# andrewjong/SwapNet

Measured on AMD Instinct MI355X. Metric: images/sec full G+D step, warp-stage 256x256 bs=32/GPU, higher is better.
Workload: dtype f32; 1 GPU; warp-stage G+D optimize_parameters step, 256x256, bs 32/GPU, fp32 storage and accumulation, GEMM products on the 16-bit MFMA pipe from operand splits: forward / input-gradient GEMMs as 2 fp16 planes of amax-scaled operands (22 of 24 mantissa bits, 3 of 4 terms, the dropped one below 2^-22), weight-gradient GEMMs in the same two-plane form, train mode (dropout 0.5), WarpModule 137.6M + PatchGAN 2.8; step_form=eager launches, global_batch=32, parallelism=dp1

## Files before the change

### swapnet_amd/csrc/wino.hip

```cpp
#include "hip_util.h"

namespace swn {
namespace {

__device__ __forceinline__ float4 f4add(float4 a, float4 b) { return make_float4(a.x + b.x, a.y + b.y, a.z + b.z, a.w + b.w); }
__device__ __forceinline__ float4 f4sub(float4 a, float4 b) { return make_float4(a.x - b.x, a.y - b.y, a.z - b.z, a.w - b.w); }

__device__ __forceinline__ int wsrc(int e, int ext, int pad_mode) {
  if (pad_mode == PAD_REFLECT) {
    if (e < 0) e = -e;
    else if (e >= ext) e = 2 * ext - 2 - e;
    return e;
  }
  return (e < 0 || e >= ext) ? -1 : e;
}

__global__ __launch_bounds__(256) void wino_input_kernel(const float* x, int xcs, int N, int H, int W, int C, int pad,
                                                         int pad_mode, int Th, int Tw, float* V) {
  const int C4 = C >> 2;
  const size_t T = (size_t)N * Th * Tw;
  const size_t total = T * C4;
  for (size_t i = (size_t)blockIdx.x * 256 + threadIdx.x; i < total; i += (size_t)gridDim.x * 256) {
    const size_t tile = i / C4;
    const int c = (int)(i - tile * C4) * 4;
// ... 378 lines not shown
#pragma unroll
    for (int b = 0; b < A; ++b) {
      float4 m[A];
#pragma unroll
      for (int a = 0; a < A; ++a) m[a] = *reinterpret_cast<const float4*>(Mx + ((size_t)(a * A + b) * T + tile) * Cm + c);
#pragma unroll
      for (int r = 0; r < M; ++r) {
        float4 s = F4ZERO;
#pragma unroll
        for (int k = 0; k < A; ++k) f4mac(s, F::AT[r][k], m[k]);
        s1[r][b] = s;
      }
    }
    float4 bv = F4ZERO;
    if (bias) bv = make_float4(c < Cout ? bias[c] : 0.f, c + 1 < Cout ? bias[c + 1] : 0.f,
                               c + 2 < Cout ? bias[c + 2] : 0.f, c + 3 < Cout ? bias[c + 3] : 0.f);
#pragma unroll
    for (int a = 0; a < M; ++a)
#pragma unroll
      for (int b = 0; b < M; ++b) {
        const int oy = M * ty + a, ox = M * tx + b;
        if (oy >= yH || ox >= yW) continue;
        float4 v = F4ZERO;
#pragma unroll
        for (int k = 0; k < A; ++k) f4mac(v, F::AT[b][k], s1[a][k]);
        v = f4add(v, bv);
        v.x = act_apply(v.x, act); v.y = act_apply(v.y, act); v.z = act_apply(v.z, act); v.w = act_apply(v.w, act);
        float* dst = y + ((size_t)(n * yH + oy) * yW + ox) * ycs + c;
        if (accumulate) v = f4add(v, *reinterpret_cast<const float4*>(dst));
        if (c + 3 < Cout) {
          *reinterpret_cast<float4*>(dst) = v;
          amx = fmaxf(amx, fmaxf(fmaxf(fabsf(v.x), fabsf(v.y)), fmaxf(fabsf(v.z), fabsf(v.w))));
        } else {
          const float vv[4] = {v.x, v.y, v.z, v.w};
          for (int j = 0; j < 4 && c + j < Cout; ++j) { dst[j] = vv[j]; amx = fmaxf(amx, fabsf(vv[j])); }
        }
      }
  }
  amax_fold(amx, amax_out);
}

template <class F, int VW>
__global__ __launch_bounds__(256) void winog_dy_kernel(const float* dy, int dcs, int N, int H, int W, int C, int Th, int Tw,
                                                       float* dM, float* amax_out, const float* in_amax, float gain, int* kscale_out) {
  constexpr int A = F::A, M = F::M;
  typedef fvec<VW> vt;
  const int Cv = C / VW;
  const size_t T = (size_t)N * Th * Tw;
  const size_t total = T * Cv;
  float am = 0.f;
  const bool pair = in_amax != nullptr;
  const float psc = pair ? __uint_as_float((unsigned)(127 + pair_scale_exp(in_amax, gain, kscale_out)) << 23) : 1.f;
  for (size_t i = (size_t)blockIdx.x * 256 + threadIdx.x; i < total; i += (size_t)gridDim.x * 256) {
    const size_t tile = i / Cv;
    const int c = (int)(i - tile * Cv) * VW;
    const int tx = (int)(tile % Tw); size_t q = tile / Tw;
    const int ty = (int)(q % Th); const int n = (int)(q / Th);
    vt r[A][M];
#pragma unroll
    for (int b = 0; b < M; ++b) {
      vt g[M];
#pragma unroll
      for (int a = 0; a < M; ++a) {
        const int oy = M * ty + a, ox = M * tx + b;
        g[a] = (oy < H && ox < W) ? *reinterpret_cast<const vt*>(dy + ((size_t)(n * H + oy) * W + ox) * dcs + c) : vt(0.f);
      }
#pragma unroll
      for (int p = 0; p < A; ++p) {
        vt s = vt(0.f);
#pragma unroll
        for (int a = 0; a < M; ++a)
          if (F::AT[a][p] != 0.f) s += F::AT[a][p] * g[a];
        r[p][b] = s;
      }
    }
#pragma unroll
    for (int p = 0; p < A; ++p)
#pragma unroll
      for (int j = 0; j < A; ++j) {
        vt s = vt(0.f);
#pragma unroll
        for (int b = 0; b < M; ++b)
          if (F::AT[b][j] != 0.f) s += F::AT[b][j] * r[p][b];
        *reinterpret_cast<vt*>(dM + ((size_t)(p * A + j) * T + tile) * C + c) = pair ? pairv<VW>(s, psc) : s;
        am = fmaxf(am, fvamax<VW>(s));
      }
  }
  if (!pair) amax_fold(am, amax_out);
}

template <class F>
__global__ __launch_bounds__(256) void winog_filter_grad_kernel(WShape w, const float* dU, float* dpacked) {
  constexpr int A = F::A, R = F::R;
  const size_t total = (size_t)w.Cip * w.Npad;
  const size_t i = (size_t)blockIdx.x * 256 + threadIdx.x;
  if (i >= total) return;
  float t[R][A];
#pragma unroll
  for (int b = 0; b < A; ++b) {
    float u[A];
#pragma unroll
    for (int a = 0; a < A; ++a) u[a] = dU[(size_t)(a * A + b) * total + i];
#pragma unroll
    for (int r = 0; r < R; ++r) {
      float s = 0.f;
#pragma unroll
      for (int a = 0; a < A; ++a) f1mac(s, F::G[a][r], u[a]);
      t[r][b] = s;
    }
  }
#pragma unroll
  for (int a = 0; a < R; ++a)
#pragma unroll
    for (int j = 0; j < R; ++j) {
      float s = 0.f;
#pragma unroll
      for (int b = 0; b < A; ++b) f1mac(s, F::G[b][j], t[a][b]);
      dpacked[(size_t)(a * R + j) * total + i] = s;
    }
}


struct F23 {
  static constexpr int M = 2, R = 3, A = 4;
  static constexpr float BT[4][4] = {{1, 0, -1, 0}, {0, 1, 1, 0}, {0, -1, 1, 0}, {0, 1, 0, -1}};
};

template <class F>
__global__ __launch_bounds__(256) void winog_patch_kernel(float* V, int C, size_t T) {
  constexpr int A = F::A;
  const int C4 = C >> 2;
  const size_t total = T * C4;
  for (size_t i = (size_t)blockIdx.x * 256 + threadIdx.x; i < total; i += (size_t)gridDim.x * 256) {
    const size_t tile = i / C4;
    const int c = (int)(i - tile * C4) * 4;
    float4 t[A][A];
#pragma unroll
    for (int b = 0; b < A; ++b) {
      float4 v[A];
#pragma unroll
      for (int a = 0; a < A; ++a) v[a] = *reinterpret_cast<const float4*>(V + ((size_t)(a * A + b) * T + tile) * C + c);
#pragma unroll
      for (int r = 0; r < A; ++r) {
        float4 s = F4ZERO;
#pragma unroll
        for (int k = 0; k < A; ++k) f4mac(s, F::BT[k][r], v[k]);
        t[r][b] = s;
      }
    }
#pragma unroll
    for (int a = 0; a < A; ++a)
#pragma unroll
      for (int j = 0; j < A; ++j) {
        float4 s = F4ZERO;
#pragma unroll
        for (int k = 0; k < A; ++k) f4mac(s, F::BT[k][j], t[a][k]);
        *reinterpret_cast<float4*>(V + ((size_t)(a * A + j) * T + tile) * C + c) = s;
      }
  }
}

__device__ __forceinline__ int adj_sources(int y, int ext, int pad, int pad_mode, int emax, int (&e)[3]) {
  int n = 0;
  if (y <= emax) e[n++] = y;
  if (pad_mode == PAD_REFLECT) {
    if (y >= 1 && -y >= -pad) e[n++] = -y;
    const int r = 2 * ext - 2 - y;
    if (r >= ext && r <= emax) e[n++] = r;
  }
  return n;
}

__global__ __launch_bounds__(256) void wino_fold_kernel(const float* P, int C, int N, int H, int W, int m, int A, int pad,
                                                        int pad_mode, int Th, int Tw, float* dx, int dcs, int accumulate) {
  const int C4 = C >> 2;
  const size_t T = (size_t)N * Th * Tw;
  const size_t total = (size_t)N * H * W * C4;
  const int emax_y = m * (Th - 1) - pad + A - 1, emax_x = m * (Tw - 1) - pad + A - 1;
  for (size_t i = (size_t)blockIdx.x * 256 + threadIdx.x; i < total; i += (size_t)gridDim.x * 256) {
    const size_t px = i / C4;
    const int c = (int)(i - px * C4) * 4;
    const int n = (int)(px / ((size_t)H * W));
    const int rem = (int)(px - (size_t)n * H * W);
    const int y = rem / W, x = rem - y * W;
    int ey[3], ex[3];
    const int ny = adj_sources(y, H, pad, pad_mode, emax_y, ey), nx = adj_sources(x, W, pad, pad_mode, emax_x, ex);
    float4 acc = F4ZERO;
    for (int iy = 0; iy < ny; ++iy) {
      const int qy = ey[iy] + pad;
      const int ty1 = min(qy / m, Th - 1);
      for (int ty = ty1; ty >= 0 && qy - m * ty < A; --ty) {
        const int a = qy - m * ty;
        for (int ix = 0; ix < nx; ++ix) {
          const int qx = ex[ix] + pad;
          const int tx1 = min(qx / m, Tw - 1);
          for (int tx = tx1; tx >= 0 && qx - m * tx < A; --tx) {
            const int b = qx - m * tx;
            const size_t tile = ((size_t)n * Th + ty) * Tw + tx;
            const float4 v = *reinterpret_cast<const float4*>(P + ((size_t)(a * A + b) * T + tile) * C + c);
            acc = f4add(acc, v);
          }
        }
      }
    }
    float* d = dx + px * dcs + c;
    if (accumulate) acc = f4add(acc, *reinterpret_cast<const float4*>(d));
    *reinterpret_cast<float4*>(d) = acc;
  }
}


struct F42 {
  static constexpr int M = 4, R = 2, A = 5;
  static constexpr float BT[5][5] = {{0.5f, -1, -0.5f, 1, 0}, {0, -0.5f, 0.5f, 1, 0}, {0, 0.5f, -1.5f, 1, 0}, {0, -1, 0, 1, 0},
                                     {0, 0.5f, -1, -0.5f, 1}};
  static constexpr float G[5][2] = {{2, 0}, {1, 1}, {-1.f / 3, 1.f / 3}, {-8.f / 3, -4.f / 3}, {0, 1}};
  static constexpr float AT[4][5] = {{1, 1, 1, 1, 0}, {0, 1, -1, 0.5f, 0}, {0, 1, 1, 0.25f, 0}, {0, 1, -1, 0.125f, 1}};
};

template <int VW>
__global__ __launch_bounds__(256) void wino_s2_input_kernel(const float* x, int xcs, int N, int H, int W, int C, int Th, int Tw,
                                                            float* V, float* amax_out, const float* in_amax, float gain, int* kscale_out) {
  constexpr int A = 5;
  typedef fvec<VW> vt;
  const int C4 = C / VW;
  const size_t T = (size_t)N * Th * Tw;
  const size_t total = T * 4 * C4;
  const int CV = 4 * C;
  float am = 0.f;
  const bool pair = in_amax != nullptr;
  const float psc = pair ? __uint_as_float((unsigned)(127 + pair_scale_exp(in_amax, gain, kscale_out)) << 23) : 1.f;
  for (size_t i = (size_t)blockIdx.x * 256 + threadIdx.x; i < total; i += (size_t)gridDim.x * 256) {
    const int c = (int)(i % C4) * VW; size_t r = i / C4;
    const int q = (int)(r & 3); const size_t tile = r >> 2;
    const int s = q >> 1, t = q & 1;
    const int tx = (int)(tile % Tw); size_t u = tile / Tw;
    const int ty = (int)(u % Th); const int n = (int)(u / Th);
    int sy[A];
#pragma unroll
    for (int a = 0; a < A; ++a) { const int e = 2 * (4 * ty + a) - 1 + s; sy[a] = (e >= 0 && e < H) ? e : -1; }
    vt tt[A][A];
#pragma unroll
    for (int b = 0; b < A; ++b) {
      const int e = 2 * (4 * tx + b) - 1 + t;
      const int sx = (e >= 0 && e < W) ? e : -1;
      vt d[A];
#pragma unroll
      for (int a = 0; a < A; ++a)
        d[a] = (sy[a] >= 0 && sx >= 0) ? *reinterpret_cast<const vt*>(x + ((size_t)(n * H + sy[a]) * W + sx) * xcs + c) : vt(0.f);
#pragma unroll
      for (int rr = 0; rr < A; ++rr) {
        vt acc = vt(0.f);
#pragma unroll
        for (int k = 0; k < A; ++k)
          if (F42::BT[rr][k] != 0.f) acc += F42::BT[rr][k] * d[k];
        tt[rr][b] = acc;
      }
    }
#pragma unroll
    for (int a = 0; a < A; ++a)
#pragma unroll
      for (int j = 0; j < A; ++j) {
        vt acc = vt(0.f);
#pragma unroll
        for (int k = 0; k < A; ++k)
          if (F42::BT[j][k] != 0.f) acc += F42::BT[j][k] * tt[a][k];
        *reinterpret_cast<vt*>(V + ((size_t)(a * A + j) * T + tile) * CV + q * C + c) = pair ? pairv<VW>(acc, psc) : acc;
        am = fmaxf(am, fvamax<VW>(acc));
      }
  }
  if (!pair) amax_fold(am, amax_out);
}

__global__ __launch_bounds__(256) void wino_s2_fold_kernel(const float* P, int C, int N, int H, int W, int Th, int Tw, const float* bias,
                                                           float* dx, int dcs, int accumulate) {
  constexpr int A = 5, M = 4;
  const int C4 = C >> 2, CV = 4 * C;
  const size_t T = (size_t)N * Th * Tw;
  const size_t total = (size_t)N * H * W * C4;
  for (size_t i = (size_t)blockIdx.x * 256 + threadIdx.x; i < total; i += (size_t)gridDim.x * 256) {
    const size_t px = i / C4;
    const int c = (int)(i - px * C4) * 4;
    const int n = (int)(px / ((size_t)H * W));
    const int rem = (int)(px - (size_t)n * H * W);
    const int r = rem / W, cc = rem - r * W;
    const int s = (r + 1) & 1, t = (cc + 1) & 1;
    const int qy = (r + 1 - s) >> 1, qx = (cc + 1 - t) >> 1;
    float4 acc = F4ZERO;
    for (int ty = min(qy / M, Th - 1); ty >= 0 && qy - M * ty < A; --ty) {
      const int a = qy - M * ty;
      for (int tx = min(qx / M, Tw - 1); tx >= 0 && qx - M * tx < A; --tx) {
        const int b = qx - M * tx;
        const size_t tile = ((size_t)n * Th + ty) * Tw + tx;
        acc = f4add(acc, *reinterpret_cast<const float4*>(P + ((size_t)(a * A + b) * T + tile) * CV + (2 * s + t) * C + c));
      }
    }
    if (bias) { acc.x += bias[c]; acc.y += bias[c + 1]; acc.z += bias[c + 2]; acc.w += bias[c + 3]; }
    float* d = dx + px * dcs + c;
    if (accumulate) acc = f4add(acc, *reinterpret_cast<const float4*>(d));
    *reinterpret_cast<float4*>(d) = acc;
  }
}

__device__ __forceinline__ size_t s2_widx(const WShape& w, int kh, int kw, int cf, int cc) {
  if (w.kind == WK_CONV) return ((size_t)(kh * 4 + kw) * w.Cip + cf) * w.Npad + cc;
  const int a = (3 - kh) & 1, dy = (3 - kh - a) >> 1, b = (3 - kw) & 1, dx = (3 - kw - b) >> 1;
  return (size_t)(a * 2 + b) * 4 * w.Cip * w.Npad + ((size_t)(dy * 2 + dx) * w.Cip + cc) * w.Npad + cf;
}

__global__ __launch_bounds__(256) void wino_s2_filter_kernel(WShape w, int mode, int Cf, int Cc, const float* packed, float* U) {
  constexpr int A = 5;
  const size_t total = (size_t)Cf * Cc;
  const size_t i = (size_t)blockIdx.x * 256 + threadIdx.x;
  if (i >= total) return;
  const int cf = mode == 0 ? (int)(i / Cc) : (int)(i % Cf), cc = mode == 0 ? (int)(i % Cc) : (int)(i / Cf);
  const size_t plane = (size_t)4 * Cf * Cc;
#pragma unroll
  for (int q = 0; q < 4; ++q) {
    const int s = q >> 1, t = q & 1;
    float g[2][2];
#pragma unroll
    for (int a = 0; a < 2; ++a)
#pragma unroll
      for (int b = 0; b < 2; ++b) g[a][b] = packed[s2_widx(w, 2 * a + s, 2 * b + t, cf, cc)];
    float tt[A][2];
#pragma unroll
    for (int r = 0; r < A; ++r)
#pragma unroll
      for (int b = 0; b < 2; ++b) tt[r][b] = F42::G[r][0] * g[0][b] + F42::G[r][1] * g[1][b];
    const size_t o = mode == 0 ? ((size_t)(q * Cf + cf) * Cc + cc) : ((size_t)cc * 4 * Cf + q * Cf + cf);
#pragma unroll
    for (int a = 0; a < A; ++a)
#pragma unroll
      for (int j = 0; j < A; ++j) U[(size_t)(a * A + j) * plane + o] = tt[a][0] * F42::G[j][0] + tt[a][1] * F42::G[j][1];
  }
}

__global__ __launch_bounds__(256) void wino_s2_filter_grad_kernel(WShape w, int Cf, int Cc, const float* dU, float* dpacked) {
  constexpr int A = 5;
  const size_t total = (size_t)Cf * Cc;
  const size_t i = (size_t)blockIdx.x * 256 + threadIdx.x;
  if (i >= total) return;
  const int cf = (int)(i / Cc), cc = (int)(i % Cc);
  const size_t plane = (size_t)4 * Cf * Cc;
#pragma unroll
  for (int q = 0; q < 4; ++q) {
    const int s = q >> 1, t = q & 1;
    const size_t o = (size_t)(q * Cf + cf) * Cc + cc;
    float tt[2][A];
#pragma unroll
    for (int b = 0; b < A; ++b) {
      float u[A];
#pragma unroll
      for (int a = 0; a < A; ++a) u[a] = dU[(size_t)(a * A + b) * plane + o];
#pragma unroll
      for (int r = 0; r < 2; ++r) {
        float acc = 0.f;
#pragma unroll
        for (int a = 0; a < A; ++a) f1mac(acc, F42::G[a][r], u[a]);
        tt[r][b] = acc;
      }
    }
#pragma unroll
    for (int a = 0; a < 2; ++a)
#pragma unroll
      for (int b = 0; b < 2; ++b) {
        float acc = 0.f;
#pragma unroll
        for (int k = 0; k < A; ++k) f1mac(acc, F42::G[k][b], tt[a][k]);
        dpacked[s2_widx(w, 2 * a + s, 2 * b + t, cf, cc)] = acc;
      }
  }
}


typedef unsigned wu32x4 __attribute__((ext_vector_type(4)));
__device__ __forceinline__ void cut8_store(const float (&u)[8], wu32x4* o, size_t e0, size_t plane_stride) {
  unsigned hi[4], mid[4], lo[4];
#pragma unroll
  for (int j = 0; j < 4; ++j) {
    const float x0 = u[2 * j], x1 = u[2 * j + 1];
    const unsigned u0 = __float_as_uint(x0), u1 = __float_as_uint(x1);
    const float r0 = x0 - __uint_as_float(u0 & 0xffff0000u), r1 = x1 - __uint_as_float(u1 & 0xffff0000u);
    const unsigned v0 = __float_as_uint(r0), v1 = __float_as_uint(r1);
    const float s0 = r0 - __uint_as_float(v0 & 0xffff0000u), s1 = r1 - __uint_as_float(v1 & 0xffff0000u);
    hi[j] = (u0 >> 16) | (u1 & 0xffff0000u);
    mid[j] = (v0 >> 16) | (v1 & 0xffff0000u);
    lo[j] = (__float_as_uint(s0) >> 16) | (__float_as_uint(s1) & 0xffff0000u);
  }
  o[e0] = wu32x4{hi[0], hi[1], hi[2], hi[3]};
  o[e0 + plane_stride] = wu32x4{mid[0], mid[1], mid[2], mid[3]};
  o[e0 + 2 * plane_stride] = wu32x4{lo[0], lo[1], lo[2], lo[3]};
}

typedef _Float16 wf16x2 __attribute__((ext_vector_type(2)));
__device__ __forceinline__ void cut8_store_h(const float (&u)[8], float sb, wu32x4* o, size_t e0, size_t plane_stride, bool low_plane) {
  unsigned hi[4], lo[4];
#pragma unroll
  for (int j = 0; j < 4; ++j) {
    const float x0 = u[2 * j] * sb, x1 = u[2 * j + 1] * sb;
    const wf16x2 hh = wf16x2{(_Float16)x0, (_Float16)x1};
    hi[j] = __builtin_bit_cast(unsigned, hh);
    lo[j] = __builtin_bit_cast(unsigned, wf16x2{(_Float16)(x0 - (float)hh[0]), (_Float16)(x1 - (float)hh[1])});
  }
  o[e0] = wu32x4{hi[0], hi[1], hi[2], hi[3]};
  if (low_plane) o[e0 + plane_stride] = wu32x4{lo[0], lo[1], lo[2], lo[3]};
}
__device__ __forceinline__ int wino_scale_exp(const float* part, int lane, int top) {
  float m = fmaxf(fmaxf(part[lane], part[lane + 64]), fmaxf(part[lane + 128], part[lane + 192]));
#pragma unroll
  for (int o = 32; o; o >>= 1) m = fmaxf(m, __shfl_xor(m, o));
  if (!(m > 0.f) || m > 3.0e38f) return 0;
  const int e = (int)((__float_as_uint(m) >> 23) & 255u) - 127;
  const int k = top - 1 - e;
  return k < -100 ? -100 : (k > 100 ? 100 : k);
}

template <class F>
__global__ __launch_bounds__(256) void winog_filter_pc_kernel(WShape w, int mode, int K, int Nn, int BN, const float* packed,
                                                              unsigned short* out, size_t panel_elems, const float* wamax, int planes) {
  constexpr int A = F::A, R = F::R;
  const int NBc = BN / 32, tiles_n = (Nn + BN - 1) / BN;
  const size_t total = (size_t)(K / 8) * tiles_n * BN;
  const size_t i = ((size_t)(blockIdx.x / (8 * A)) * 8 + blockIdx.x % 8) * 256 + threadIdx.x;
  const int PL = planes;
  int kB = 0;
  if (wamax) kB = wino_scale_exp(wamax, threadIdx.x & 63, 10);
  if (i >= total) return;
  const int nl = (int)(i % BN); const size_t q = i / BN;
  const int tn = (int)(q % tiles_n), kq = (int)(q / tiles_n);
  const int n = tn * BN + nl;
  const int pos = (nl % NBc) * 32 + nl / NBc;
  const int a = (int)(blockIdx.x % (8 * A)) / 8;
  float Ga[R];
#pragma unroll
  for (int qq = 0; qq < R; ++qq) Ga[qq] = F::G[a][qq];
  float t[8][R];
#pragma unroll
  for (int kk = 0; kk < 8; ++kk)
#pragma unroll
    for (int b = 0; b < R; ++b) t[kk][b] = 0.f;
  if (mode == 0) {
    if (n < w.Npad) {
#pragma unroll
      for (int kk = 0; kk < 8; ++kk) {
        const int k = kq * 8 + kk;
        if (k < w.Cip) {
#pragma unroll
          for (int qq = 0; qq < R; ++qq)
#pragma unroll
            for (int b = 0; b < R; ++b) t[kk][b] += Ga[qq] * packed[((size_t)(qq * R + b) * w.Cip + k) * w.Npad + n];
        }
      }
    }
  } else if (n < w.Cip && kq * 8 < w.Npad) {
#pragma unroll
    for (int qq = 0; qq < R; ++qq)
#pragma unroll
      for (int b = 0; b < R; ++b) {
        const int tap = mode == 1 ? (R - 1 - qq) * R + (R - 1 - b) : qq * R + b;
        const float4* src = reinterpret_cast<const float4*>(packed + ((size_t)tap * w.Cip + n) * w.Npad + kq * 8);
        const float4 g0 = src[0], g1 = src[1];
        t[0][b] += Ga[qq] * g0.x; t[1][b] += Ga[qq] * g0.y; t[2][b] += Ga[qq] * g0.z; t[3][b] += Ga[qq] * g0.w;
        t[4][b] += Ga[qq] * g1.x; t[5][b] += Ga[qq] * g1.y; t[6][b] += Ga[qq] * g1.z; t[7][b] += Ga[qq] * g1.w;
      }
  }
  const size_t e0 = ((((size_t)(kq >> 1) * tiles_n + tn) * 2 + (kq & 1)) * PL) * BN + pos;
  const float sb = __uint_as_float((unsigned)(127 + kB) << 23);
#pragma unroll
  for (int j = 0; j < A; ++j) {
    float u[8];
#pragma unroll
    for (int kk = 0; kk < 8; ++kk) {
      float s = 0.f;
#pragma unroll
      for (int qq = 0; qq < R; ++qq) f1mac(s, F::G[j][qq], t[kk][qq]);
      u[kk] = s;
    }
    unsigned short* panel = out + (size_t)(a * A + j) * panel_elems;
    if (wamax) {
      cut8_store_h(u, sb, reinterpret_cast<wu32x4*>(panel), e0, (size_t)BN, PL == 2);
      if (i == 0) *reinterpret_cast<int*>(panel + (size_t)(K / 16) * tiles_n * 2 * PL * BN * 8) = kB;
    } else {
      cut8_store(u, reinterpret_cast<wu32x4*>(panel), e0, (size_t)BN);
    }
  }
}


__device__ __forceinline__ size_t tailw_fold_off(int Cip, int Npad, int ph) {
  const int pre = ph == 0 ? 0 : (ph == 1 ? 4 : (ph == 2 ? 10 : 16));
  return (size_t)pre * Cip * Npad;
}
__global__ __launch_bounds__(256) void tailw_filter_kernel(int Cip, int Npad, const float* folded, float* U) {
  constexpr int A = 6, R = 3;
  const int N4 = 4 * Npad;
  const size_t total = (size_t)Cip * N4;
  const size_t i = (size_t)blockIdx.x * 256 + threadIdx.x;
  if (i >= total) return;
  const int ci = (int)(i / N4), n = (int)(i % N4);
  const int ph = n / Npad, co = n - ph * Npad, a = ph >> 1, b = ph & 1;
  const float* f = folded + tailw_fold_off(Cip, Npad, ph);
  float g[R][R];
#pragma unroll
  for (int r = 0; r < R; ++r)
#pragma unroll
    for (int c = 0; c < R; ++c) g[r][c] = (r < 2 + a && c < 2 + b) ? f[((size_t)(r * (2 + b) + c) * Cip + ci) * Npad + co] : 0.f;
  float t[A][R];
#pragma unroll
  for (int r = 0; r < A; ++r)
#pragma unroll
    for (int c = 0; c < R; ++c) {
      float s = 0.f;
#pragma unroll
      for (int q = 0; q < R; ++q) f1mac(s, F43::G[r][q], g[q][c]);
      t[r][c] = s;
    }
#pragma unroll
  for (int r = 0; r < A; ++r)
#pragma unroll
    for (int j = 0; j < A; ++j) {
      float s = 0.f;
#pragma unroll
      for (int q = 0; q < R; ++q) f1mac(s, F43::G[j][q], t[r][q]);
      U[(size_t)(r * A + j) * total + i] = s;
    }
}
__global__ __launch_bounds__(256) void tailw_filter_grad_kernel(int Cip, int Npad, const float* dU, float* dfolded) {
  constexpr int A = 6, R = 3;
  const int N4 = 4 * Npad;
  const size_t total = (size_t)Cip * N4;
  const size_t i = (size_t)blockIdx.x * 256 + threadIdx.x;
  if (i >= total) return;
  const int ci = (int)(i / N4), n = (int)(i % N4);
  const int ph = n / Npad, co = n - ph * Npad, a = ph >> 1, b = ph & 1;
  float t[R][A];
#pragma unroll
  for (int j = 0; j < A; ++j) {
    float u[A];
#pragma unroll
    for (int r = 0; r < A; ++r) u[r] = dU[(size_t)(r * A + j) * total + i];
#pragma unroll
    for (int q = 0; q < R; ++q) {
      float s = 0.f;
#pragma unroll
      for (int r = 0; r < A; ++r) f1mac(s, F43::G[r][q], u[r]);
      t[q][j] = s;
    }
  }
  float* f = dfolded + tailw_fold_off(Cip, Npad, ph);
#pragma unroll
  for (int r = 0; r < R; ++r)
#pragma unroll
    for (int c = 0; c < R; ++c) {
      if (r >= 2 + a || c >= 2 + b) continue;
      float s = 0.f;
#pragma unroll
      for (int j = 0; j < A; ++j) f1mac(s, F43::G[j][c], t[r][j]);
      f[((size_t)(r * (2 + b) + c) * Cip + ci) * Npad + co] = s;
    }
}
__global__ __launch_bounds__(256) void tailw_output_kernel(const float* Mx, int N, int Th, int Tw, int Npad, const float* bias, int act,
                                                           float* y, int ycs, int yH, int yW, int Cout) {
  constexpr int A = 6, M = 4;
  const int C4 = Npad >> 2, CM = 4 * Npad;
  const size_t T = (size_t)N * Th * Tw;
  const size_t total = T * 4 * C4;
  for (size_t i = (size_t)blockIdx.x * 256 + threadIdx.x; i < total; i += (size_t)gridDim.x * 256) {
    const int c = (int)(i % C4) * 4; size_t r = i / C4;
    const int ph = (int)(r & 3); const size_t tile = r >> 2;
    const int a = ph >> 1, b = ph & 1;
    const int tx = (int)(tile % Tw); size_t u = tile / Tw;
    const int ty = (int)(u % Th); const int n = (int)(u / Th);
    float4 s1[M][A];
#pragma unroll
    for (int j = 0; j < A; ++j) {
      float4 m[A];
#pragma unroll
      for (int k = 0; k < A; ++k) m[k] = *reinterpret_cast<const float4*>(Mx + ((size_t)(k * A + j) * T + tile) * CM + ph * Npad + c);
#pragma unroll
      for (int q = 0; q < M; ++q) {
        float4 s = F4ZERO;
#pragma unroll
        for (int k = 0; k < A; ++k) f4mac(s, F43::AT[q][k], m[k]);
        s1[q][j] = s;
      }
    }
    float4 bv = F4ZERO;
    if (bias) bv = make_float4(c < Cout ? bias[c] : 0.f, c + 1 < Cout ? bias[c + 1] : 0.f, c + 2 < Cout ? bias[c + 2] : 0.f,
                               c + 3 < Cout ? bias[c + 3] : 0.f);
#pragma unroll
    for (int q = 0; q < M; ++q)
#pragma unroll
      for (int jj = 0; jj < M; ++jj) {
        const int oy = 2 * (M * ty + q) + a, ox = 2 * (M * tx + jj) + b;
        if (oy >= yH || ox >= yW) continue;
        float4 v = F4ZERO;
#pragma unroll
        for (int k = 0; k < A; ++k) f4mac(v, F43::AT[jj][k], s1[q][k]);
        v = f4add(v, bv);
        v.x = act_apply(v.x, act); v.y = act_apply(v.y, act); v.z = act_apply(v.z, act); v.w = act_apply(v.w, act);
        float* dst = y + ((size_t)(n * yH + oy) * yW + ox) * ycs + c;
        if (c + 3 < Cout) {
          *reinterpret_cast<float4*>(dst) = v;
        } else {
          const float vv[4] = {v.x, v.y, v.z, v.w};
          for (int e = 0; e < 4 && c + e < Cout; ++e) dst[e] = vv[e];
        }
      }
  }
}
__global__ __launch_bounds__(256) void tailw_dy_kernel(const float* dy, int dcs, int N, int yH, int yW, int Th, int Tw, int Npad,
                                                       float* dM, float* amax_out, const float* in_amax, float gain, int* kscale_out) {
  constexpr int A = 6, M = 4;
  const int C4 = Npad >> 2, CM = 4 * Npad;
  const size_t T = (size_t)N * Th * Tw;
  const size_t total = T * 4 * C4;
  float am = 0.f;
  const bool pair = in_amax != nullptr;
  const float psc = pair ? __uint_as_float((unsigned)(127 + pair_scale_exp(in_amax, gain, kscale_out)) << 23) : 1.f;
  for (size_t i = (size_t)blockIdx.x * 256 + threadIdx.x; i < total; i += (size_t)gridDim.x * 256) {
    const int c = (int)(i % C4) * 4; size_t r = i / C4;
    const int ph = (int)(r & 3); const size_t tile = r >> 2;
    const int a = ph >> 1, b = ph & 1;
    const int tx = (int)(tile % Tw); size_t u = tile / Tw;
    const int ty = (int)(u % Th); const int n = (int)(u / Th);
    float4 rr[A][M];
#pragma unroll
    for (int jj = 0; jj < M; ++jj) {
      float4 g[M];
#pragma unroll
      for (int q = 0; q < M; ++q) {
        const int oy = 2 * (M * ty + q) + a, ox = 2 * (M * tx + jj) + b;
        g[q] = (oy < yH && ox < yW) ? *reinterpret_cast<const float4*>(dy + ((size_t)(n * yH + oy) * yW + ox) * dcs + c) : F4ZERO;
      }
#pragma unroll
      for (int p = 0; p < A; ++p) {
        float4 s = F4ZERO;
#pragma unroll
        for (int q = 0; q < M; ++q) f4mac(s, F43::AT[q][p], g[q]);
        rr[p][jj] = s;
      }
    }
#pragma unroll
    for (int p = 0; p < A; ++p)
#pragma unroll
      for (int j = 0; j < A; ++j) {
        float4 s = F4ZERO;
#pragma unroll
        for (int jj = 0; jj < M; ++jj) f4mac(s, F43::AT[jj][j], rr[p][jj]);
        *reinterpret_cast<float4*>(dM + ((size_t)(p * A + j) * T + tile) * CM + ph * Npad + c) = pair ? pair4(s, psc) : s;
        am = fmaxf(am, f4amax(s));
      }
  }
  if (!pair) amax_fold(am, amax_out);
}

inline unsigned wgrid(size_t total) { return (unsigned)std::min<size_t>(std::max<size_t>((total + 255) / 256, 1), 256 * 32); }

}

static int variant(int m, int r) {
  if (m == 2 && r == 3) return 0;
  if (m == 4 && r == 3) return 1;
  if (m == 3 && r == 4) return 2;
  if (m == 4 && r == 2) return 3;
  throw Error(1, "winograd: supported forms are F(2,3), F(4,3), F(3,4) and the strided F(4,2)");
}
static constexpr int wino_vec_width() { return 2; }
static float input_gain(int v) { return v == 3 ? 9.f : 100.f; }
static float dy_gain(int v) { return v == 1 ? 225.f : (v == 2 ? 49.f : 16.f); }
void wino_input_transform(Stream& s, int m, int r, const TView& x, int pad, int pad_mode, int Th, int Tw, float* V, float* amax_out,
                          const float* in_amax, int* kscale_out) {
  const int v = variant(m, r);
  if (v == 3) throw Error(1, "wino_input_transform: F(4,2) is the strided form (wino_s2_input_transform)");
  if (x.C % 4 || x.cs % 4) throw Error(1, "wino_input_transform: C must be a multiple of 4");
  const int vw = wino_vec_width();
  const size_t total = (size_t)x.N * Th * Tw * (x.C / (v == 0 ? 4 : vw));
  const dim3 grid(wgrid(total));
  if (v == 0 && in_amax) throw Error(1, "wino_input_transform: F(2,3) planes have no pair form");
#define SWN_WIN_LAUNCH(F, VW)                                                                                                  \
  hipLaunchKernelGGL((winog_input_kernel<F, VW>), grid, dim3(256), 0, hs(s), x.p, x.cs, x.N, x.H, x.W, x.C, pad, pad_mode, Th, \
                     Tw, V, amax_out, in_amax, input_gain(v), kscale_out)
  if (v == 0)
    hipLaunchKernelGGL(wino_input_kernel, grid, dim3(256), 0, hs(s), x.p, x.cs, x.N, x.H, x.W, x.C, pad, pad_mode, Th, Tw, V);
  else if (v == 1) SWN_WIN_LAUNCH(F43, 2);
  else SWN_WIN_LAUNCH(F34, 2);
#undef SWN_WIN_LAUNCH
  check_launch("wino_input_transform");
}
void wino_filter_transform(Stream& s, int m, int r, const WShape& w, int mode, const float* packed, float* U) {
  const int v = variant(m, r);
  if (v == 3) throw Error(1, "wino_filter_transform: F(4,2) is the strided form (wino_s2_filter_transform)");
  const int K = mode == 0 ? w.Cip : w.Npad, Nn = mode == 0 ? w.Npad : w.Cip;
  const dim3 grid((unsigned)(((size_t)K * Nn + 255) / 256));
  if (v == 0) hipLaunchKernelGGL(wino_filter_kernel, grid, dim3(256), 0, hs(s), w, mode, K, Nn, packed, U);
  else if (v == 1) hipLaunchKernelGGL(winog_filter_kernel<F43>, grid, dim3(256), 0, hs(s), w, mode, K, Nn, packed, U);
  else hipLaunchKernelGGL(winog_filter_kernel<F34>, grid, dim3(256), 0, hs(s), w, mode, K, Nn, packed, U);
  check_launch("wino_filter_transform");
}
void wino_filter_transform_pc(Stream& s, int m, int r, const WShape& w, int mode, const float* packed, int bn, uint16_t* out,
                              size_t panel_elems, const float** amax_io) {
  const int v = variant(m, r);
  if (v != 1 && v != 2) throw Error(1, "wino_filter_transform_pc: the 6-point forms F(4,3) / F(3,4) only");
  if (mode < 0 || mode > 2) throw Error(1, "wino_filter_transform_pc: mode 0, 1 or 2");
  const int K = mode == 0 ? w.Cip : w.Npad, Nn = mode == 0 ? w.Npad : w.Cip;
  if (K % 16 || (bn != 64 && bn != 128)) throw Error(1, "wino_filter_transform_pc: K must be a multiple of 16, tile 64 or 128");
  const size_t total = (size_t)(K / 8) * ((Nn + bn - 1) / bn) * bn;
  const dim3 grid((unsigned)((((total + 255) / 256 + 7) / 8) * 8) * (unsigned)(m + r - 1));
  const float* wamax = (amax_io && *amax_io) ? *amax_io : conv_precut_amax(s, packed, (size_t)r * r * w.Cip, w.Npad, 1, 0);
  if (amax_io) *amax_io = wamax;
  if (v == 1)
    hipLaunchKernelGGL(winog_filter_pc_kernel<F43>, grid, dim3(256), 0, hs(s), w, mode, K, Nn, bn, packed, out, panel_elems, wamax,
                       conv_precut_planes());
  else
    hipLaunchKernelGGL(winog_filter_pc_kernel<F34>, grid, dim3(256), 0, hs(s), w, mode, K, Nn, bn, packed, out, panel_elems, wamax,
                       conv_precut_planes());
  check_launch("wino_filter_transform_pc");
}
void wino_output_transform(Stream& s, int m, int r, const float* M, int Cm, int Th, int Tw, const float* bias, int act,
                           const TView& y, int Cout, int accumulate, float* amax_out) {
  const int v = variant(m, r);
  if (v == 0 && amax_out) throw Error(1, "wino_output_transform: the F(2,3) kernel has no amax fold");
  const size_t total = (size_t)y.N * Th * Tw * ((Cout + 3) / 4);
  const dim3 grid(wgrid(total));
  if (v == 0)
    hipLaunchKernelGGL(wino_output_kernel, grid, dim3(256), 0, hs(s), M, Cm, y.N, Th, Tw, bias, act, y.p, y.cs, y.H, y.W,
                       Cout, accumulate);
  else if (v == 1)
    hipLaunchKernelGGL(winog_output_kernel<F43>, grid, dim3(256), 0, hs(s), M, Cm, y.N, Th, Tw, bias, act, y.p, y.cs, y.H,
                       y.W, Cout, accumulate, amax_out);
  else if (v == 2)
    hipLaunchKernelGGL(winog_output_kernel<F34>, grid, dim3(256), 0, hs(s), M, Cm, y.N, Th, Tw, bias, act, y.p, y.cs, y.H,
                       y.W, Cout, accumulate, amax_out);
  else
    hipLaunchKernelGGL(winog_output_kernel<F42>, grid, dim3(256), 0, hs(s), M, Cm, y.N, Th, Tw, bias, act, y.p, y.cs, y.H,
                       y.W, Cout, accumulate, amax_out);
  check_launch("wino_output_transform");
}
void wino_dy_transform(Stream& s, int m, int r, const TView& dy, int Th, int Tw, float* dM, float* amax_out, const float* in_amax,
                       int* kscale_out) {
  const int v = variant(m, r);
  if (dy.C % 4 || dy.cs % 4) throw Error(1, "wino_dy_transform: C must be a multiple of 4");
  const int vw = v == 0 ? 4 : wino_vec_width();
  const size_t total = (size_t)dy.N * Th * Tw * (dy.C / vw);
  const dim3 grid(wgrid(total));
  if (v == 0 && in_amax) throw Error(1, "wino_dy_transform: F(2,3) planes have no pair form");
#define SWN_WDY_LAUNCH(F, VW)                                                                                                       \
  hipLaunchKernelGGL((winog_dy_kernel<F, VW>), grid, dim3(256), 0, hs(s), dy.p, dy.cs, dy.N, dy.H, dy.W, dy.C, Th, Tw, dM, amax_out, \
                     in_amax, dy_gain(v), kscale_out)
  if (v == 0)
    hipLaunchKernelGGL(wino_dy_kernel, grid, dim3(256), 0, hs(s), dy.p, dy.cs, dy.N, dy.H, dy.W, dy.C, Th, Tw, dM);
  else if (v == 1) SWN_WDY_LAUNCH(F43, 2);
  else if (v == 2) SWN_WDY_LAUNCH(F34, 2);
  else SWN_WDY_LAUNCH(F42, 2);
#undef SWN_WDY_LAUNCH
  check_launch("wino_dy_transform");
}
void tailw_filter_transform(Stream& s, const WShape& w, const float* folded, float* U) {
  const size_t total = (size_t)w.Cip * 4 * w.Npad;
  hipLaunchKernelGGL(tailw_filter_kernel, dim3((unsigned)((total + 255) / 256)), dim3(256), 0, hs(s), w.Cip, w.Npad, folded, U);
  check_launch("tailw_filter_transform");
}
void tailw_filter_grad(Stream& s, const WShape& w, const float* dU, float* dfolded) {
  const size_t total = (size_t)w.Cip * 4 * w.Npad;
  hipLaunchKernelGGL(tailw_filter_grad_kernel, dim3((unsigned)((total + 255) / 256)), dim3(256), 0, hs(s), w.Cip, w.Npad, dU, dfolded);
  check_launch("tailw_filter_grad");
}
void tailw_output_transform(Stream& s, const float* M, int Th, int Tw, int Npad, const float* bias, int act, const TView& y, int Cout) {
  if (Npad % 4 || y.cs % 4 || y.C < Npad) throw Error(1, "tailw_output_transform: bad channel counts");
  const size_t total = (size_t)y.N * Th * Tw * 4 * (Npad / 4);
  hipLaunchKernelGGL(tailw_output_kernel, dim3(wgrid(total)), dim3(256), 0, hs(s), M, y.N, Th, Tw, Npad, bias, act, y.p, y.cs, y.H, y.W, Cout);
  check_launch("tailw_output_transform");
}
void tailw_dy_transform(Stream& s, const TView& dy, int Th, int Tw, int Npad, float* dM, float* amax_out, const float* in_amax,
                        int* kscale_out) {
  if (Npad % 4 || dy.cs % 4 || dy.C < Npad) throw Error(1, "tailw_dy_transform: bad channel counts");
  const size_t total = (size_t)dy.N * Th * Tw * 4 * (Npad / 4);
  hipLaunchKernelGGL(tailw_dy_kernel, dim3(wgrid(total)), dim3(256), 0, hs(s), dy.p, dy.cs, dy.N, dy.H, dy.W, Th, Tw, Npad, dM, amax_out,
                     in_amax, 225.f, kscale_out);
  check_launch("tailw_dy_transform");
}
void wino_s2_input_transform(Stream& s, const TView& x, int Th, int Tw, float* V, float* amax_out, const float* in_amax, int* kscale_out) {
  if (x.C % 4 || x.cs % 4) throw Error(1, "wino_s2_input_transform: C must be a multiple of 4");
  const int vw = wino_vec_width();
  const size_t total = (size_t)x.N * Th * Tw * 4 * (x.C / vw);
  hipLaunchKernelGGL(wino_s2_input_kernel<2>, dim3(wgrid(total)), dim3(256), 0, hs(s), x.p, x.cs, x.N, x.H, x.W, x.C, Th, Tw, V,
                       amax_out, in_amax, 9.f, kscale_out);
  check_launch("wino_s2_input_transform");
}
void wino_s2_input_adjoint(Stream& s, float* dV, int Cf, int Th, int Tw, const TView& dx, const float* bias, int accumulate) {
  if (Cf % 4 || dx.C != Cf || dx.cs % 4) throw Error(1, "wino_s2_input_adjoint: bad channel count");
  const size_t T = (size_t)dx.N * Th * Tw;
  hipLaunchKernelGGL(winog_patch_kernel<F42>, dim3(wgrid(T * Cf)), dim3(256), 0, hs(s), dV, 4 * Cf, T);
  hipLaunchKernelGGL(wino_s2_fold_kernel, dim3(wgrid(dx.pixels() * (Cf / 4))), dim3(256), 0, hs(s), dV, Cf, dx.N, dx.H, dx.W, Th, Tw,
                     bias, dx.p, dx.cs, accumulate);
  check_launch("wino_s2_input_adjoint");
}
static void s2_dims(const WShape& w, int& Cf, int& Cc) {
  if (w.KH != 4 || w.KW != 4) throw Error(1, "strided Winograd: k4 s2 layers only");
  Cf = w.kind == WK_CONV ? w.Cip : w.Npad;
  Cc = w.kind == WK_CONV ? w.Npad : w.Cip;
}
void wino_s2_filter_transform(Stream& s, const WShape& w, int mode, const float* packed, float* U) {
  int Cf, Cc;
  s2_dims(w, Cf, Cc);
  hipLaunchKernelGGL(wino_s2_filter_kernel, dim3((unsigned)(((size_t)Cf * Cc + 255) / 256)), dim3(256), 0, hs(s), w, mode, Cf, Cc, packed, U);
  check_launch("wino_s2_filter_transform");
}
void wino_s2_filter_grad(Stream& s, const WShape& w, const float* dU, float* dpacked) {
  int Cf, Cc;
  s2_dims(w, Cf, Cc);
  hipLaunchKernelGGL(wino_s2_filter_grad_kernel, dim3((unsigned)(((size_t)Cf * Cc + 255) / 256)), dim3(256), 0, hs(s), w, Cf, Cc, dU, dpacked);
  check_launch("wino_s2_filter_grad");
}
void wino_input_adjoint(Stream& s, int m, int r, float* dV, int C, int pad, int pad_mode, int Th, int Tw, const TView& dx,
                        int accumulate) {
  const int v = variant(m, r);
  if (v == 3) throw Error(1, "wino_input_adjoint: F(4,2) is the strided form (wino_s2_input_adjoint)");
  if (C % 4 || dx.C != C || dx.cs % 4) throw Error(1, "wino_input_adjoint: bad channel count");
  const size_t T = (size_t)dx.N * Th * Tw;
  const dim3 grid(wgrid(T * (C / 4)));
  if (v == 0) hipLaunchKernelGGL(winog_patch_kernel<F23>, grid, dim3(256), 0, hs(s), dV, C, T);
  else if (v == 1) hipLaunchKernelGGL(winog_patch_kernel<F43>, grid, dim3(256), 0, hs(s), dV, C, T);
  else hipLaunchKernelGGL(winog_patch_kernel<F34>, grid, dim3(256), 0, hs(s), dV, C, T);
  const int A = m + r - 1;
  hipLaunchKernelGGL(wino_fold_kernel, dim3(wgrid(dx.pixels() * (C / 4))), dim3(256), 0, hs(s), dV, C, dx.N, dx.H, dx.W, m, A, pad,
                     pad_mode, Th, Tw, dx.p, dx.cs, accumulate);
  check_launch("wino_input_adjoint");
}
void wino_filter_grad(Stream& s, int m, int r, const WShape& w, const float* dU, float* dpacked) {
  const int v = variant(m, r);
  if (v == 3) throw Error(1, "wino_filter_grad: F(4,2) is the strided form (wino_s2_filter_grad)");
  const size_t total = (size_t)w.Cip * w.Npad;
  const dim3 grid((unsigned)((total + 255) / 256));
  if (v == 0) hipLaunchKernelGGL(wino_filter_grad_kernel, grid, dim3(256), 0, hs(s), w, dU, dpacked);
  else if (v == 1) hipLaunchKernelGGL(winog_filter_grad_kernel<F43>, grid, dim3(256), 0, hs(s), w, dU, dpacked);
  else hipLaunchKernelGGL(winog_filter_grad_kernel<F34>, grid, dim3(256), 0, hs(s), w, dU, dpacked);
  check_launch("wino_filter_grad");
}

}
```

Measured before the change: 1340 images/sec.

## Fuse Winograd input-adjoint output transform and fold into one LDS-staged kernel

Replaces the two-kernel Winograd input-gradient adjoint (in-place output transform of dV, then a gather fold into dx) with a single kernel. Each block transforms a band of tile rows into LDS, keeps the overlapping halo rows in a double-buffered carry region, and folds directly into dx with bias and accumulate. This removes a full write and reread of the transformed dV tensor in global memory plus one launch, for both the F(4,3) and strided F(4,2) paths. In exchange it needs up to 80 KB of dynamic LDS per block, which limits occupancy, and it adds a planner that falls back to the old path for unsupported shapes.

```diff
diff --git a/swapnet_amd/csrc/wino.hip b/swapnet_amd/csrc/wino.hip
--- a/swapnet_amd/csrc/wino.hip
+++ b/swapnet_amd/csrc/wino.hip
@@ -704,6 +704,175 @@
   }
 }
 
+struct AdjPlan {
+  int rows = 0;
+  int single = 0;
+  int bands = 1, band_rows = 0;
+  size_t lds = 0;
+};
+constexpr size_t ADJ_LDS_BUDGET = 80 * 1024;
+
+template <class F, bool S2>
+__global__ __launch_bounds__(256) void wino_adjoint_onepass_kernel(const float* __restrict__ V, int Cv, int C, int N, int H, int W, int Th,
+                                                                   int Tw, int pad, int pad_mode, int rows, int single, int bands,
+                                                                   int band_rows, int units, const float* __restrict__ bias,
+                                                                   float* dx, int dcs, int accumulate) {
+  constexpr int A = F::A, M = F::M, E = A * A, OV = A - M;
+  constexpr int L = S2 ? 16 : 8;
+  constexpr int LP = S2 ? 4 : 8;
+  extern __shared__ float4 adj_lds[];
+  float4* const mainb = adj_lds;
+  float4* const carry = adj_lds + (size_t)rows * Tw * E * L;
+  const int carry_n = Tw * OV * A * L;
+
+  int u = blockIdx.x, c0;
+  if (S2) {
+    u = (blockIdx.x >> 4) * 8 + (blockIdx.x & 7);
+    if (u >= units) return;
+    const int GP = C >> 5;
+    c0 = (u % GP) * 32 + ((blockIdx.x >> 3) & 1) * 16;
+    u /= GP;
+  } else {
+    const int G = C >> 5;
+    c0 = (u % G) * 32;
+    u /= G;
+  }
+  const int band = u % bands, n = u / bands;
+  const int ty0 = band * band_rows, ty1 = min(ty0 + band_rows, Th);
+  const size_t T = (size_t)N * Th * Tw;
+  const int emax_y = M * (Th - 1) - pad + A - 1, emax_x = M * (Tw - 1) - pad + A - 1;
+  const int tid = threadIdx.x;
+
+  int k = 0;
+  for (int tyA = ty0 > 0 ? ty0 - 1 : 0; tyA < ty1; ++k) {
+    const bool halo = tyA < ty0;
+    const int nr = halo ? 1 : min(rows, ty1 - tyA);
+    float4* const cur = carry + (k & 1) * carry_n;
+    const float4* const prev = carry + ((k & 1) ^ 1) * carry_n;
+    for (int it = tid; it < nr * Tw * L; it += 256) {
+      const int lane = it % L, tl = it / L;
+      const int tx = tl % Tw, r = tl / Tw;
+      const size_t tile = ((size_t)n * Th + tyA + r) * Tw + tx;
+      const int c = S2 ? (lane >> 2) * C + c0 + (lane & 3) * 4 : c0 + lane * 4;
+      float4 t[A][A];
+#pragma unroll
+      for (int b = 0; b < A; ++b) {
+        float4 v[A];
+#pragma unroll
+        for (int a = 0; a < A; ++a) v[a] = *reinterpret_cast<const float4*>(V + ((size_t)(a * A + b) * T + tile) * Cv + c);
+#pragma unroll
+        for (int rr = 0; rr < A; ++rr) {
+          float4 s = F4ZERO;
+#pragma unroll
+          for (int kk = 0; kk < A; ++kk) f4mac(s, F::BT[kk][rr], v[kk]);
+          t[rr][b] = s;
+        }
+      }
+      float4* const mt = mainb + (size_t)(r * Tw + tx) * E * L + lane;
+      float4* const ct = cur + (size_t)tx * OV * A * L + lane;
+      const bool to_carry = !single && r == nr - 1;
+#pragma unroll
+      for (int a = 0; a < A; ++a)
+#pragma unroll
+        for (int j = 0; j < A; ++j) {
+          float4 s = F4ZERO;
+#pragma unroll
+          for (int kk = 0; kk < A; ++kk) f4mac(s, F::BT[kk][j], t[a][kk]);
+          if (a >= M && to_carry) ct[((a - M) * A + j) * L] = s;
+          else mt[(a * A + j) * L] = s;
+        }
+    }
+    __syncthreads();
+    if (!halo) {
+      const int qlo = M * tyA, qhi = (tyA + nr == Th) ? M * (Th - 1) + A : M * (tyA + nr);
+      const int ya = S2 ? max(2 * qlo - 1, 0) : max(qlo - pad, 0);
+      const int yb = S2 ? min(2 * qhi - 1, H) : min(qhi - pad, H);
+      auto at = [&](int ty, int tx, int a, int b, int lane) -> float4 {
+        const int r = ty - tyA;
+        if (r < 0) return prev[((size_t)tx * OV * A + (a - M) * A + b) * L + lane];
+        if (!single && r == nr - 1 && a >= M) return cur[((size_t)tx * OV * A + (a - M) * A + b) * L + lane];
+        return mainb[((size_t)(r * Tw + tx) * E + a * A + b) * L + lane];
+      };
+      for (int it = tid; it < (yb - ya) * W * LP; it += 256) {
+        const int lp = it % LP, px = it / LP;
+        const int x = px % W, y = ya + px / W;
+        const int c = c0 + lp * 4;
+        float4 acc = F4ZERO;
+        if (S2) {
+          const int s = (y + 1) & 1, tt = (x + 1) & 1;
+          const int qy = (y + 1 - s) >> 1, qx = (x + 1 - tt) >> 1;
+          const int lane = (2 * s + tt) * 4 + lp;
+          for (int ty = min(qy / M, Th - 1); ty >= 0 && qy - M * ty < A; --ty) {
+            const int a = qy - M * ty;
+            for (int tx = min(qx / M, Tw - 1); tx >= 0 && qx - M * tx < A; --tx) acc = f4add(acc, at(ty, tx, a, qx - M * tx, lane));
+          }
+          if (bias) { acc.x += bias[c]; acc.y += bias[c + 1]; acc.z += bias[c + 2]; acc.w += bias[c + 3]; }
+        } else {
+          int ey[3], ex[3];
+          const int ny = adj_sources(y, H, pad, pad_mode, emax_y, ey), nx = adj_sources(x, W, pad, pad_mode, emax_x, ex);
+          for (int iy = 0; iy < ny; ++iy) {
+            const int qy = ey[iy] + pad;
+            for (int ty = min(qy / M, Th - 1); ty >= 0 && qy - M * ty < A; --ty) {
+              const int a = qy - M * ty;
+              for (int ix = 0; ix < nx; ++ix) {
+                const int qx = ex[ix] + pad;
+                for (int tx = min(qx / M, Tw - 1); tx >= 0 && qx - M * tx < A; --tx) acc = f4add(acc, at(ty, tx, a, qx - M * tx, lp));
+              }
+            }
+          }
+        }
+        float* d = dx + (((size_t)n * H + y) * W + x) * dcs + c;
+        if (accumulate) acc = f4add(acc, *reinterpret_cast<const float4*>(d));
+        *reinterpret_cast<float4*>(d) = acc;
+      }
+      __syncthreads();
+    }
+    tyA += nr;
+  }
+}
+
+AdjPlan adjoint_plan(int v, int C, int N, int H, int W, int pad, int Th, int Tw) {
+  AdjPlan p;
+  const bool s2 = v == 3;
+  if (v != 1 && !s2) return p;
+  if (C % 32 || Th < 1 || Tw < 1) return p;
+  if (!s2 && (pad != 1 || H != 4 * Th || W != 4 * Tw)) return p;
+  if (s2 && (H > 8 * Th + 1 || W > 8 * Tw + 1)) return p;
+  const int A = s2 ? 5 : 6, M = 4, L = s2 ? 16 : 8;
+  const size_t row = (size_t)Tw * A * A * L * 16, carry = (size_t)2 * Tw * (A - M) * A * L * 16;
+  if ((size_t)Th * row <= ADJ_LDS_BUDGET) {
+    p.rows = Th; p.single = 1; p.bands = 1; p.band_rows = Th; p.lds = (size_t)Th * row;
+    return p;
+  }
+  if (row + carry > ADJ_LDS_BUDGET) return p;
+  p.rows = (int)((ADJ_LDS_BUDGET - carry) / row);
+  p.lds = (size_t)p.rows * row + carry;
+  const int steps = (Th + p.rows - 1) / p.rows;
+  const size_t blocks = (size_t)N * (C / (s2 ? 16 : 32));
+  const int want = (int)std::min<size_t>((512 + blocks - 1) / blocks, (size_t)steps);
+  p.band_rows = ((steps + want - 1) / want) * p.rows;
+  p.bands = (Th + p.band_rows - 1) / p.band_rows;
+  return p;
+}
+
+template <class F, bool S2>
+void adjoint_onepass_launch(Stream& s, const AdjPlan& p, const float* dV, int Cv, int C, int pad, int pad_mode, int Th, int Tw,
+                            const TView& dx, const float* bias, int accumulate) {
+  auto* kern = wino_adjoint_onepass_kernel<F, S2>;
+  static bool attr_set[64] = {};
+  int dev = 0;
+  if (hipGetDevice(&dev) != hipSuccess || dev < 0 || dev >= 64) throw Error(1, "wino adjoint: no current device");
+  if (!attr_set[dev]) {
+    if (hipFuncSetAttribute(reinterpret_cast<const void*>(kern), hipFuncAttributeMaxDynamicSharedMemorySize, (int)ADJ_LDS_BUDGET) != hipSuccess)
+      throw Error(1, "wino adjoint: cannot raise the dynamic LDS limit");
+    attr_set[dev] = true;
+  }
+  const int units = dx.N * p.bands * (C / 32);
+  const unsigned grid = S2 ? (unsigned)((units + 7) / 8) * 16 : (unsigned)units;
+  hipLaunchKernelGGL(kern, dim3(grid), dim3(256), p.lds, hs(s), dV, Cv, C, dx.N, dx.H, dx.W, Th, Tw, pad, pad_mode, p.rows, p.single, p.bands,
+                     p.band_rows, units, bias, dx.p, dx.cs, accumulate);
+}
+
 __device__ __forceinline__ size_t s2_widx(const WShape& w, int kh, int kw, int cf, int cc) {
   if (w.kind == WK_CONV) return ((size_t)(kh * 4 + kw) * w.Cip + cf) * w.Npad + cc;
   const int a = (3 - kh) & 1, dy = (3 - kh - a) >> 1, b = (3 - kw) & 1, dx = (3 - kw - b) >> 1;
@@ -1194,9 +1363,14 @@
 void wino_s2_input_adjoint(Stream& s, float* dV, int Cf, int Th, int Tw, const TView& dx, const float* bias, int accumulate) {
   if (Cf % 4 || dx.C != Cf || dx.cs % 4) throw Error(1, "wino_s2_input_adjoint: bad channel count");
   const size_t T = (size_t)dx.N * Th * Tw;
-  hipLaunchKernelGGL(winog_patch_kernel<F42>, dim3(wgrid(T * Cf)), dim3(256), 0, hs(s), dV, 4 * Cf, T);
-  hipLaunchKernelGGL(wino_s2_fold_kernel, dim3(wgrid(dx.pixels() * (Cf / 4))), dim3(256), 0, hs(s), dV, Cf, dx.N, dx.H, dx.W, Th, Tw,
-                     bias, dx.p, dx.cs, accumulate);
+  const AdjPlan plan = adjoint_plan(3, Cf, dx.N, dx.H, dx.W, 1, Th, Tw);
+  if (plan.rows) {
+    adjoint_onepass_launch<F42, true>(s, plan, dV, 4 * Cf, Cf, 1, PAD_ZERO, Th, Tw, dx, bias, accumulate);
+  } else {
+    hipLaunchKernelGGL(winog_patch_kernel<F42>, dim3(wgrid(T * Cf)), dim3(256), 0, hs(s), dV, 4 * Cf, T);
+    hipLaunchKernelGGL(wino_s2_fold_kernel, dim3(wgrid(dx.pixels() * (Cf / 4))), dim3(256), 0, hs(s), dV, Cf, dx.N, dx.H, dx.W, Th, Tw,
+                       bias, dx.p, dx.cs, accumulate);
+  }
   check_launch("wino_s2_input_adjoint");
 }
 static void s2_dims(const WShape& w, int& Cf, int& Cc) {
@@ -1222,6 +1396,12 @@
   if (v == 3) throw Error(1, "wino_input_adjoint: F(4,2) is the strided form (wino_s2_input_adjoint)");
   if (C % 4 || dx.C != C || dx.cs % 4) throw Error(1, "wino_input_adjoint: bad channel count");
   const size_t T = (size_t)dx.N * Th * Tw;
+  const AdjPlan plan = adjoint_plan(v, C, dx.N, dx.H, dx.W, pad, Th, Tw);
+  if (plan.rows) {
+    adjoint_onepass_launch<F43, false>(s, plan, dV, C, C, pad, pad_mode, Th, Tw, dx, nullptr, accumulate);
+    check_launch("wino_input_adjoint");
+    return;
+  }
   const dim3 grid(wgrid(T * (C / 4)));
   if (v == 0) hipLaunchKernelGGL(winog_patch_kernel<F23>, grid, dim3(256), 0, hs(s), dV, C, T);
   else if (v == 1) hipLaunchKernelGGL(winog_patch_kernel<F43>, grid, dim3(256), 0, hs(s), dV, C, T);
```

Result: slower. 1318 images/sec (-1.7%).
